# bartelvdh/Navtex

Hardware: AMD Instinct MI355X
Metric: IQ Msamples/s through FIR->FSK->bitsync (higher is better)
Workload: dtype f64

## Files before the change

navtex_amd/csrc/nvx_cascade.hip:

```cpp
#include <hip/hip_runtime.h>
#include <stdint.h>
#include <stdlib.h>
#include <mutex>

#include "nvx_cascade_wave.h"
#include "nvx_tune_table.h"

__device__ double2 nvx_tune_tab[NVX_TUNE_TAB_ENTRIES];

__device__ __forceinline__ int add_low_halves(unsigned a, unsigned b)
{
    int r;
    asm("v_add_u32_sdwa %0, sext(%1), sext(%2) dst_sel:DWORD dst_unused:UNUSED_PAD src0_sel:WORD_0 src1_sel:WORD_0"
        : "=v"(r) : "v"(a), "v"(b));
    return r;
}
__device__ __forceinline__ int add_high_halves(unsigned a, unsigned b)
{
    int r;
    asm("v_add_u32_sdwa %0, sext(%1), sext(%2) dst_sel:DWORD dst_unused:UNUSED_PAD src0_sel:WORD_1 src1_sel:WORD_1"
        : "=v"(r) : "v"(a), "v"(b));
    return r;
}
__device__ __forceinline__ double stage0_component(u32x4 v, bool odd)
{
    const int sI = add_low_halves(v.x, v.y) + add_low_halves(v.z, v.w);
    const int sQ = add_high_halves(v.x, v.y) + add_high_halves(v.z, v.w);
    int mine = (odd ? sQ : sI) + 4;
    const int other = odd ? sI : sQ;
    asm("" : "+v"(mine));
    const int tot = mine + dpp_swap_pairs(other);
    return (double)(tot >> 3);
}

struct Stage0Cic3 {
    unsigned sel_mine, sel_other;
    unsigned wa0, wa1, wb0, wb1, wc0, wc1;
    int c_prev, t_prev;
    bool last_pair;

    __device__ __forceinline__ void init(int lane)
    {
        const bool odd = lane & 1;
        sel_mine = odd ? 0x07060302u : 0x05040100u;
        sel_other = odd ? 0x05040100u : 0x07060302u;
        wa0 = odd ? (10u | 6u << 16) : (36u | 28u << 16);  wa1 = odd ? (3u | 1u << 16) : (21u | 15u << 16);
        wb0 = odd ? (48u | 48u << 16) : (28u | 36u << 16); wb1 = odd ? (46u | 42u << 16) : (42u | 46u << 16);
        wc0 = odd ? (6u | 10u << 16) : 0u;                 wc1 = odd ? (15u | 21u << 16) : (1u | 3u << 16);
        last_pair = lane >= 62;
        c_prev = 0; t_prev = 0;
    }
    __device__ __forceinline__ static int rot1(int v) { return __builtin_amdgcn_mov_dpp(v, 0x13C, 0xF, 0xF, false); }
    __device__ __forceinline__ static void dot2_first(nvx_short2 a, unsigned wb, unsigned wc, int &b, int &c)
    {
        asm("v_dot2_i32_i16 %0, %2, %3, 0\n\t"
            "v_dot2_i32_i16 %1, %2, %4, 0\n\t"
            "s_nop 2"
            : "=&v"(b), "=v"(c) : "v"(a), "v"(wb), "v"(wc));
    }
    __device__ __forceinline__ double step(u32x4 v)
    {
        const nvx_short2 m01 = as_short2(__builtin_amdgcn_perm(v.y, v.x, sel_mine)), m23 = as_short2(__builtin_amdgcn_perm(v.w, v.z, sel_mine));
        const nvx_short2 o01 = as_short2(__builtin_amdgcn_perm(v.y, v.x, sel_other)), o23 = as_short2(__builtin_amdgcn_perm(v.w, v.z, sel_other));
        int oa = __builtin_amdgcn_sdot2(o01, as_short2(wa0), 256, false); oa = __builtin_amdgcn_sdot2(o23, as_short2(wa1), oa, false);
        int ob, oc;
        dot2_first(o01, wb0, wc0, ob, oc);
        ob = __builtin_amdgcn_sdot2(o23, as_short2(wb1), ob, false); oc = __builtin_amdgcn_sdot2(o23, as_short2(wc1), oc, false);
        int A = dpp_swap_pairs(oa); A = __builtin_amdgcn_sdot2(m01, as_short2(wa0), A, false); A = __builtin_amdgcn_sdot2(m23, as_short2(wa1), A, false);
        int B = dpp_swap_pairs(ob); B = __builtin_amdgcn_sdot2(m01, as_short2(wb0), B, false); B = __builtin_amdgcn_sdot2(m23, as_short2(wb1), B, false);
        int C = dpp_swap_pairs(oc); C = __builtin_amdgcn_sdot2(m01, as_short2(wc0), C, false); C = __builtin_amdgcn_sdot2(m23, as_short2(wc1), C, false);
        const int t = B + rot1(rot1(last_pair ? c_prev : C));
        const int y = A + rot1(rot1(last_pair ? t_prev : t));
        c_prev = C; t_prev = t;
        return (double)(y >> 9);
    }
};

template <bool RAW>
__device__ __forceinline__ void load_pass(u32x4 (&pf)[RAW ? 8 : 1], const u32x4 *src)
{
    if (RAW) {
#pragma unroll
        for (int j = 0; j < 8; j++) pf[j] = __builtin_nontemporal_load(src + 64 * j);
    } else {
        pf[0] = __builtin_nontemporal_load(src);
    }
}

#define NVX_SPIN_LIMIT (1 << 22)

template <bool RAW, int NCH, int S0, typename ARGS, bool LIST = false>
__device__ __forceinline__ void cascade_wave_main(ARGS a)
{
    __shared__ CascadeLds<NCH> lds;
    const int lane = threadIdx.x;
    CascadeWave<NCH> cw;
    cw.init(&lds, lane);

    const size_t pass_words = RAW ? 2048 : 256;
    const size_t pass_stride = pass_words / 4;
    constexpr int NPF = RAW ? 8 : 1;
    const int half = lane >> 1, comp = lane & 1;
    const bool odd = lane & 1;
    double *xw = (double *)&lds.X[(half & 7) * XS + XH + (lane >> 4)] + comp;
    double2 *xw4 = &lds.X[(lane & 1) * 4 * XS + XH + half];
    static_assert(S0 == 1 || (S0 == 3 && RAW), "the third-order stage 0 belongs to the raw-rate kernels");
    Stage0Cic3 s0;
    if (S0 == 3) s0.init(lane);
    const int n_full = a.n_streams * a.split_from;
    const int n_units = n_full + 3 * a.n_streams * (a.n_frames - a.split_from);

    for (;;) {
        int u = 0;
        if (lane == 0) u = __hip_atomic_fetch_add(a.queue, 1, __ATOMIC_RELAXED, __HIP_MEMORY_SCOPE_AGENT);
        u = __builtin_amdgcn_readfirstlane(u);
        if (u >= n_units) break;
        int tpart, thirds, entry;
        if (u < n_full) { const int frame = u / a.n_streams; entry = u - frame * a.n_streams; tpart = 3 * frame; thirds = 3; }
        else { const int v = u - n_full, q = v / a.n_streams; entry = v - q * a.n_streams; tpart = 3 * a.split_from + q; thirds = 1; }
        const int part = tpart;
        int stream = entry;
        const uint8_t *state_rd = a.state[0];
        uint8_t *state_wr = a.state[1];
        unsigned third0 = a.third0;
        if (LIST) {
            const unsigned long long e = nvx_load_const_u64(a.part + entry);
            stream = (int)(unsigned)e;
            if (e >> 32) { state_rd = a.state[1]; state_wr = a.state[0]; }
            third0 = (unsigned)(nvx_load_const_u64(&a.part[entry].g0) / NVX_THIRD_Y3);
        }
        int *const done = a.done + entry;
        const unsigned mask = a.chain_masks[stream];

        bool preroll = a.independent && part > 0;
        bool late_publish = false;
        const u32x4 *unit0 = (const u32x4 *)(a.iq + ((size_t)stream * a.pitch + a.first_sample)) + (size_t)part * NVX_THIRD_PASSES * pass_stride + lane;
        u32x4 pfA[NPF];
        if (!preroll) load_pass<RAW>(pfA, unit0);

        if (part > 0 && !a.independent) {
            int spins = 0, ok = 0;
            do {
                int d = 0;
                if (lane == 0) d = __hip_atomic_load(done, __ATOMIC_RELAXED, __HIP_MEMORY_SCOPE_AGENT);
                d = __builtin_amdgcn_readfirstlane(d);
                ok = d >= part;
                if (!ok && a.dynamic_preroll) break;
                if (!ok) __builtin_amdgcn_s_sleep(32);
            } while (!ok && ++spins < NVX_SPIN_LIMIT);
            if (!ok && a.dynamic_preroll) {
                preroll = true; late_publish = true;
                if (lane == 0) __hip_atomic_fetch_add(a.status + 2, 1, __ATOMIC_RELAXED, __HIP_MEMORY_SCOPE_AGENT);
            } else {
                if (spins > 0 && lane == 0) {
                    __hip_atomic_fetch_add(a.status + 1, spins, __ATOMIC_RELAXED, __HIP_MEMORY_SCOPE_AGENT);
                    __hip_atomic_fetch_add(a.status + 2, 1, __ATOMIC_RELAXED, __HIP_MEMORY_SCOPE_AGENT);
                }
                if (!ok) {
                    if (lane == 0) __hip_atomic_store(a.status, NVX_STATUS_TIMEOUT, __ATOMIC_RELAXED, __HIP_MEMORY_SCOPE_AGENT);
                    break;
                }
                asm volatile("" ::: "memory");
            }
        }

        double2 *st = (double2 *)(state_wr + (size_t)stream * NVX_CASCADE_STATE_BYTES);
        const double2 *st_in = (part == 0) ? (const double2 *)(state_rd + (size_t)stream * NVX_CASCADE_STATE_BYTES) : st;
#ifdef NVX_INJECT_STALE
        if (part > 0 && !preroll && (u % NVX_INJECT_STALE) == 0) st_in = (const double2 *)(state_rd + (size_t)stream * NVX_CASCADE_STATE_BYTES);
#endif
        cw.set_mask(mask);
        unsigned long long ct = 0;
        if (!preroll) {
            NVX_WAVE_LDS_FENCE();
            const unsigned long long sealed = seal_load(st_in);
            unsigned long long fold = cw.state_in(st_in);
            if (S0 == 3 && s0.last_pair) {
                ct = __hip_atomic_load((const unsigned long long *)(st_in + NVX_STATE_CIC3) + (lane & 1), __ATOMIC_RELAXED, __HIP_MEMORY_SCOPE_AGENT);
                fold ^= seal_rotc<37>(ct);
            }
            const unsigned third_in = third0 + (unsigned)part;
            if (third_in != 0 && !seal_ok(sealed, wave_fold64(fold), stream, third_in)) {
                if (part == 0) {
                    if (lane == 0) __hip_atomic_store(a.status, NVX_STATUS_INTEGRITY, __ATOMIC_RELAXED, __HIP_MEMORY_SCOPE_AGENT);
                } else {
                    preroll = true; ct = 0;
                    if (lane == 0) __hip_atomic_fetch_add(a.status + 3, 1, __ATOMIC_RELAXED, __HIP_MEMORY_SCOPE_AGENT);
                }
            }
        }
        const int pre = preroll ? NVX_PREROLL_PASSES : 0;
        const int n_pass = pre + thirds * NVX_THIRD_PASSES;
        const u32x4 *src = unit0 - (size_t)pre * pass_stride;
        if (preroll) load_pass<RAW>(pfA, src);
        const u32x4 *nxt = src + pass_stride;
        cw.begin_unit(mask, a.y3, (size_t)(stream * 2) * a.y3_cap + a.y3_base + (size_t)part * NVX_THIRD_Y3, a.y3_cap,
                      ((part % 3) * (NVX_THIRD_PASSES * 64)) % NVX_MIX_N,
                      preroll ? NVX_PREROLL_U : 0, preroll ? NVX_PREROLL_Y2 : 0, !preroll);
        NVX_WAVE_LDS_FENCE();
        if (preroll) cw.state_zero();
        NVX_WAVE_LDS_FENCE();
        if (S0 == 3) { s0.c_prev = (int)(unsigned)ct; s0.t_prev = (int)(unsigned)(ct >> 32); }
        {
            const unsigned long long k01 = nvx_load_const_u64(a.tune_k + 2 * stream);
            int o_first = (part % 3) * (NVX_THIRD_PASSES * 64) - pre * 64;
            if (o_first < 0) o_first += NVX_PASSES_PER_FRAME * 64;
            cw.begin_table_mix((int)(unsigned)k01, (int)(unsigned)(k01 >> 32), o_first);
        }

        auto body = [&](u32x4 (&pf)[NPF], const int pass) {
            cw.tune_fetch(nvx_tune_tab);
            if (RAW) {
#pragma unroll
                for (int j = 0; j < 8; j++) xw[j * 8] = (S0 == 3) ? s0.step(pf[j]) : stage0_component(pf[j], odd);
            } else {
                const uint32_t w[4] = { pf[0].x, pf[0].y, pf[0].z, pf[0].w };
#pragma unroll
                for (int r = 0; r < 4; r++) {
                    double2 v;
                    v.x = (double)(int)(short)(w[r] & 0xffffu);
                    v.y = (double)((int)w[r] >> 16);
                    xw4[r * XS] = v;
                }
            }
            cw.tune_ready();
            if (pass + 1 < n_pass) load_pass<RAW>(pf, nxt);
            nxt += pass_stride;
            NVX_WAVE_LDS_FENCE();
            cw.compute_pass(true);
        };

        for (int pass = 0; pass < n_pass; pass++) {
            if (pass == pre) { cw.emit = true; cw.n3_done = 0; }
            body(pfA, pass);
        }

        NVX_WAVE_LDS_FENCE();
        if (late_publish) {
            int spins = 0, ok = 0;
            do {
                int d = 0;
                if (lane == 0) d = __hip_atomic_load(done, __ATOMIC_RELAXED, __HIP_MEMORY_SCOPE_AGENT);
                d = __builtin_amdgcn_readfirstlane(d);
                ok = d >= part;
                if (!ok) __builtin_amdgcn_s_sleep(32);
            } while (!ok && ++spins < NVX_SPIN_LIMIT);
            if (spins > 0 && lane == 0) __hip_atomic_fetch_add(a.status + 1, spins, __ATOMIC_RELAXED, __HIP_MEMORY_SCOPE_AGENT);
            if (!ok) {
                if (lane == 0) __hip_atomic_store(a.status, NVX_STATUS_TIMEOUT, __ATOMIC_RELAXED, __HIP_MEMORY_SCOPE_AGENT);
                break;
            }
            asm volatile("" ::: "memory");
        }
        if (!a.independent || part + thirds == 3 * a.n_frames) {
            unsigned long long fold = cw.state_out(st);
            if (S0 == 3 && s0.last_pair) {
                const unsigned long long ct_out = (unsigned long long)(unsigned)s0.c_prev | ((unsigned long long)(unsigned)s0.t_prev << 32);
                __hip_atomic_store((unsigned long long *)(st + NVX_STATE_CIC3) + (lane & 1), ct_out, __ATOMIC_RELAXED, __HIP_MEMORY_SCOPE_AGENT);
                fold ^= seal_rotc<37>(ct_out);
            }
            fold = wave_fold64(fold);
            if (lane == 0) seal_store(st, fold, stream, third0 + (unsigned)(part + thirds));
        }
        asm volatile("s_waitcnt vmcnt(0)" ::: "memory");
        if (lane == 0 && !a.independent) __hip_atomic_store(done, part + thirds, __ATOMIC_RELAXED, __HIP_MEMORY_SCOPE_AGENT);
    }
}

template <bool RAW, int NCH>
__global__ __launch_bounds__(64) void nvx_fir_cascade(nvx_cascade_args a)
{
    if (RAW) cascade_wave_main<RAW, NCH, 1, const nvx_cascade_args &>(a);
    else cascade_wave_main<RAW, NCH, 1, const nvx_cascade_args>(a);
}

__global__ __launch_bounds__(64) __attribute__((amdgpu_waves_per_eu(3, 3))) void nvx_fir_cascade_cic3_1(nvx_cascade_args a) { cascade_wave_main<true, 1, 3, const nvx_cascade_args &>(a); }
__global__ __launch_bounds__(64) void nvx_fir_cascade_cic3_2(nvx_cascade_args a) { cascade_wave_main<true, 2, 3, const nvx_cascade_args &>(a); }

template <bool RAW, int NCH, int S0>
__global__ __launch_bounds__(64) void nvx_fir_cascade_list(nvx_cascade_args a)
{
    if (RAW) cascade_wave_main<RAW, NCH, S0, const nvx_cascade_args &, true>(a);
    else cascade_wave_main<RAW, NCH, S0, const nvx_cascade_args, true>(a);
}

template <bool RAW, int NCH, int S0, bool LIST> struct CascadeKernel { static constexpr auto fn = nvx_fir_cascade_list<RAW, NCH, S0>; };
template <bool RAW, int NCH> struct CascadeKernel<RAW, NCH, 1, false> { static constexpr auto fn = nvx_fir_cascade<RAW, NCH>; };
template <> struct CascadeKernel<true, 1, 3, false> { static constexpr auto fn = nvx_fir_cascade_cic3_1; };
template <> struct CascadeKernel<true, 2, 3, false> { static constexpr auto fn = nvx_fir_cascade_cic3_2; };

#define NVX_MAX_DEVICES 64
static int env_int(const char *name, int dflt) { const char *e = getenv(name); return e ? atoi(e) : dflt; }

template <bool RAW, int NCH, int S0 = 1, bool LIST = false>
static hipError_t launch_cascade_as(const nvx_cascade_args *a, hipStream_t s)
{
    static std::mutex mu;
    static int cus_of[NVX_MAX_DEVICES], fit_of[NVX_MAX_DEVICES];
    int n_cus = 0, fit_per_cu = 0;
    {
        int dev = 0;
        hipError_t e = hipGetDevice(&dev);
        if (e != hipSuccess) return e;
        std::lock_guard<std::mutex> lk(mu);
        const bool cached = dev >= 0 && dev < NVX_MAX_DEVICES && cus_of[dev] > 0;
        if (!cached) {
            int cus = 0, per_cu = 0;
            e = hipDeviceGetAttribute(&cus, hipDeviceAttributeMultiprocessorCount, dev);
            if (e == hipSuccess) e = hipOccupancyMaxActiveBlocksPerMultiprocessor(&per_cu, CascadeKernel<RAW, NCH, S0, LIST>::fn, 64, 0);
            if (e != hipSuccess) return e;
            n_cus = cus; fit_per_cu = per_cu > 0 ? per_cu : 1;
            if (dev >= 0 && dev < NVX_MAX_DEVICES) { cus_of[dev] = n_cus; fit_of[dev] = fit_per_cu; }
        } else {
            n_cus = cus_of[dev]; fit_per_cu = fit_of[dev];
        }
    }
    int per_cu = fit_per_cu;
    if (a->max_waves_per_cu > 0 && a->max_waves_per_cu < per_cu) per_cu = a->max_waves_per_cu;
    if (a->max_waves_per_cu < 0 && per_cu + a->max_waves_per_cu >= 4) per_cu += a->max_waves_per_cu;
    const int resident = n_cus * per_cu;
    nvx_cascade_args args = *a;
    static const int force = env_int("NVX_INDEPENDENT", -1);
    args.independent = force >= 0 ? force : (a->n_streams < resident && a->n_frames > 1);
    const long long whole_units = (long long)a->n_streams * a->n_frames;
    const int split_frames = whole_units > resident ? 1 : ((args.independent && 3 * whole_units <= resident) ? a->n_frames : 0);
    args.split_from = a->n_frames - split_frames;
    const long long units = (long long)a->n_streams * (args.split_from + 3LL * split_frames);
    const unsigned grid = (unsigned)(units < resident ? units : resident);
    static const int dynamic = env_int("NVX_DYNAMIC_PREROLL", 1);
    args.dynamic_preroll = dynamic != 0;
    hipLaunchKernelGGL((CascadeKernel<RAW, NCH, S0, LIST>::fn), dim3(grid), dim3(64), 0, s, args);
    return hipGetLastError();
}

static hipError_t tune_table_ready()
{
    static std::mutex mu;
    static bool done[NVX_MAX_DEVICES];
    int dev = 0;
    hipError_t e = hipGetDevice(&dev);
    if (e != hipSuccess) return e;
    if (dev < 0 || dev >= NVX_MAX_DEVICES) return hipErrorInvalidDevice;
    std::lock_guard<std::mutex> lk(mu);
    if (done[dev]) return hipSuccess;
    double2 *tab = (double2 *)calloc(NVX_TUNE_TAB_ENTRIES, sizeof(double2));
    if (!tab) return hipErrorOutOfMemory;
    for (int j = 0; j < NVX_TUNE_TAB_N; j++) nvx_tune_entry(j, &tab[j].x, &tab[j].y);
    for (int o = 0; o < NVX_MIX_N; o++) {
        const int j = (NVX_TUNE_NOMINAL_K * o) % NVX_TUNE_TAB_N;
        tab[NVX_TUNE_TAB_N + j] = double2{ NVX_MIX_CR[o], NVX_MIX_CI[o] };
        tab[2 * NVX_TUNE_TAB_N + (NVX_TUNE_TAB_N - j) % NVX_TUNE_TAB_N] = double2{ NVX_MIX_CR[o], -NVX_MIX_CI[o] };
    }
    e = hipMemcpyToSymbol(HIP_SYMBOL(nvx_tune_tab), tab, NVX_TUNE_TAB_ENTRIES * sizeof(double2), 0, hipMemcpyHostToDevice);
    free(tab);
    if (e == hipSuccess) done[dev] = true;
    return e;
}

extern "C" hipError_t nvx_launch_cascade(const nvx_cascade_args *a, int raw, int nch, hipStream_t s)
{
    { hipError_t e = tune_table_ready(); if (e != hipSuccess) return e; }
    hipError_t e = hipMemsetAsync(a->queue, 0, (size_t)(NVX_CASCADE_CTRL_INTS + a->n_streams) * sizeof(int), s);
    if (e != hipSuccess) return e;
    const bool cic3 = raw && a->stage0_order == 3;
    if (a->part) {
        if (cic3) return nch == 1 ? launch_cascade_as<true, 1, 3, true>(a, s) : launch_cascade_as<true, 2, 3, true>(a, s);
        if (raw) return nch == 1 ? launch_cascade_as<true, 1, 1, true>(a, s) : launch_cascade_as<true, 2, 1, true>(a, s);
        return nch == 1 ? launch_cascade_as<false, 1, 1, true>(a, s) : launch_cascade_as<false, 2, 1, true>(a, s);
    }
    if (cic3) return nch == 1 ? launch_cascade_as<true, 1, 3>(a, s) : launch_cascade_as<true, 2, 3>(a, s);
    if (raw) return nch == 1 ? launch_cascade_as<true, 1>(a, s) : launch_cascade_as<true, 2>(a, s);
    return nch == 1 ? launch_cascade_as<false, 1>(a, s) : launch_cascade_as<false, 2>(a, s);
}
```

navtex_amd/csrc/nvx_cascade_wave.h:

```cpp
#ifndef NVX_CASCADE_WAVE_H
#define NVX_CASCADE_WAVE_H

#include <hip/hip_runtime.h>
#include <stdint.h>

#include "nvx_tables.h"
#include "nvx_kernels.h"
#include "nvx_device.h"

#define XPH 8
#define XH 5
#define XS 37
#define X_ENTRIES (XPH * XS)
#define NVX_Y2_RUN 160

template <int NCH> struct Geo;
template <> struct Geo<1> { static constexpr int U_RUN = 224, Y2_PER_RUN = 32, Y2_RUN = NVX_Y2_RUN, Y3_PER_RUN = NVX_Y2_RUN / 10, U_PEND_MAX = 256, U_LEFT_MAX = 32; };
template <> struct Geo<2> { static constexpr int U_RUN = 112, Y2_PER_RUN = 16, Y2_RUN = 80, Y3_PER_RUN = 8, U_PEND_MAX = 160, U_LEFT_MAX = 48; };
template <int NCH> struct GeoSizes {
    static constexpr int U_ENTRIES = ((46 + Geo<NCH>::U_PEND_MAX) + 7) / 8 * 8;
    static constexpr int Y2_ENTRIES = ((70 + Geo<NCH>::Y2_RUN) + 7) / 8 * 8;
};
static_assert(Geo<1>::Y2_RUN % Geo<1>::Y2_PER_RUN == 0 && Geo<2>::Y2_RUN % Geo<2>::Y2_PER_RUN == 0, "NVX_Y2_RUN: a whole number of FIR2 runs (160)");
static_assert(Geo<1>::U_RUN % 32 == 0 && Geo<2>::U_RUN % 16 == 0 && 46 + Geo<1>::U_LEFT_MAX <= 128 && 46 + Geo<2>::U_LEFT_MAX <= 128, "slide covers two rows of 64");

template <int NCH, bool F3IN> struct CascadeLdsY2 { double2 Y2[NCH][GeoSizes<NCH>::Y2_ENTRIES]; };
template <int NCH> struct CascadeLdsY2<NCH, false> {};
template <int NCH, bool F3IN = true>
struct CascadeLds : CascadeLdsY2<NCH, F3IN> {
    double2 X[X_ENTRIES];
    double2 U[NCH][GeoSizes<NCH>::U_ENTRIES];
    double2 mix[2][2 * NVX_MIX_N];
};

__device__ __forceinline__ int dpp_swap_pairs(int v)
{
    return __builtin_amdgcn_mov_dpp(v, 0xB1, 0xF, 0xF, true);
}
__device__ __forceinline__ double dpp_swap_pairs_f64(double v)
{
    return __hiloint2double(dpp_swap_pairs(__double2hiint(v)), dpp_swap_pairs(__double2loint(v)));
}

#define NVX_F1_GROUP 4
#define NVX_F1_AHEAD 3
#define NVX_F23_AHEAD 12
__device__ __forceinline__ constexpr int f1_offset(int j)
{
    const int t = 7 - j, r = t & 7, fl = (t - r) / 8;
    return 2 * (r * XS + fl);
}

template <int N> struct TapIndex {
    int first[N];
    constexpr TapIndex(const double (&h)[N]) : first{}
    {
        for (int i = 0; i < N; i++) {
            int f = i;
            for (int k = 0; k < i; k++) if (h[k] == h[i]) { f = k; break; }
            first[i] = f;
        }
    }
};
static constexpr TapIndex<NVX_T1> NVX_H1_FIRST(NVX_H1);

__device__ __forceinline__ double2 state_load(const double2 *p)
{
    double2 r;
    r.x = __hip_atomic_load(&p->x, __ATOMIC_RELAXED, __HIP_MEMORY_SCOPE_AGENT);
    r.y = __hip_atomic_load(&p->y, __ATOMIC_RELAXED, __HIP_MEMORY_SCOPE_AGENT);
    return r;
}
__device__ __forceinline__ void state_store(double2 *p, double2 v)
{
    __hip_atomic_store(&p->x, v.x, __ATOMIC_RELAXED, __HIP_MEMORY_SCOPE_AGENT);
    __hip_atomic_store(&p->y, v.y, __ATOMIC_RELAXED, __HIP_MEMORY_SCOPE_AGENT);
}

template <int R> __device__ __forceinline__ unsigned long long seal_rotc(unsigned long long v)
{
    constexpr int r = R & 63;
    if constexpr (r == 0) return v;
    else return (v << r) | (v >> (64 - r));
}
template <int SLOT> __device__ __forceinline__ unsigned long long seal_pair(double2 v)
{
    return seal_rotc<14 * SLOT + 3>((unsigned long long)__double_as_longlong(v.x)) ^ seal_rotc<14 * SLOT + 10>((unsigned long long)__double_as_longlong(v.y));
}
__device__ __forceinline__ unsigned long long seal_tag(int stream, unsigned third)
{
    unsigned long long t = ((unsigned long long)(unsigned)stream << 32) | third;
    t *= 0x9E3779B97F4A7C15ull; t ^= t >> 29; t *= 0xBF58476D1CE4E5B9ull; t ^= t >> 32;
    return t;
}
template <int CTRL, int R> __device__ __forceinline__ unsigned long long seal_step(unsigned long long v)
{
    const unsigned lo = (unsigned)__builtin_amdgcn_mov_dpp((int)(unsigned)v, CTRL, 0xF, 0xF, true);
    const unsigned hi = (unsigned)__builtin_amdgcn_mov_dpp((int)(unsigned)(v >> 32), CTRL, 0xF, 0xF, true);
    return v ^ seal_rotc<R>(((unsigned long long)hi << 32) | lo);
}
__device__ __forceinline__ unsigned long long seal_row(unsigned lo, unsigned hi, int lane0)
{
    return ((unsigned long long)(unsigned)__builtin_amdgcn_readlane((int)hi, lane0) << 32) | (unsigned)__builtin_amdgcn_readlane((int)lo, lane0);
}
__device__ __forceinline__ unsigned long long wave_fold64(unsigned long long v)
{
    v = seal_step<0xB1, 1>(v);
    v = seal_step<0x4E, 2>(v);
    v = seal_step<0x141, 4>(v);
    v = seal_step<0x140, 8>(v);
    const unsigned lo = (unsigned)v, hi = (unsigned)(v >> 32);
    return seal_row(lo, hi, 0) ^ seal_rotc<16>(seal_row(lo, hi, 16)) ^ seal_rotc<32>(seal_row(lo, hi, 32)) ^ seal_rotc<48>(seal_row(lo, hi, 48));
}
__device__ __forceinline__ void seal_store(double2 *st, unsigned long long fold, int stream, unsigned third)
{
    unsigned long long *p = (unsigned long long *)(st + NVX_STATE_SEAL);
    __hip_atomic_store(p, fold ^ seal_tag(stream, third), __ATOMIC_RELAXED, __HIP_MEMORY_SCOPE_AGENT);
    __hip_atomic_store(p + 1, ((unsigned long long)(unsigned)stream << 32) | third, __ATOMIC_RELAXED, __HIP_MEMORY_SCOPE_AGENT);
}
__device__ __forceinline__ unsigned long long seal_load(const double2 *st_in)
{
    return __hip_atomic_load((const unsigned long long *)(st_in + NVX_STATE_SEAL), __ATOMIC_RELAXED, __HIP_MEMORY_SCOPE_AGENT);
}
__device__ __forceinline__ bool seal_ok(unsigned long long got, unsigned long long fold, int stream, unsigned third)
{
    const unsigned long long d = got ^ fold ^ seal_tag(stream, third);
    return __builtin_amdgcn_readfirstlane((int)((unsigned)d | (unsigned)(d >> 32))) == 0;
}

template <int NCH, bool F3IN = true>
struct CascadeWave {
    CascadeLds<NCH, F3IN> *lds;
    int lane, half, comp;
    const lds_vdouble *xrv;
    const lds_vd2 *mixrow;
    int lane_mod9;
    double h1v[NVX_T1];
    unsigned mask;
    int chain_of_slot0;
    int n_u, n_y2, n3_done, mixbase;
    nvx_d2 mix_next;
    bool emit;
    double2 *y3; size_t y3_row0, y3_cap;
    double2 *y2_lane; int n2_done;
    int toff[NCH], tk[NCH], tidx[NCH];
    nvx_d2 tc[NCH];

    __device__ __forceinline__ void init(CascadeLds<NCH, F3IN> *l, int lane_)
    {
        lds = l; lane = lane_; half = lane >> 1; comp = lane & 1;
        xrv = (const lds_vdouble *)((const double *)&lds->X[XH + half] + comp);
        lane_mod9 = (2 * half) % 9;
        if (!F3IN && lane < 4 * NVX_MIX_N) {
            const int j9 = lane % NVX_MIX_N;
            double cr = 0.0, ci = 0.0;
#pragma unroll
            for (int j = 0; j < NVX_MIX_N; j++) if (j9 == j) { cr = NVX_MIX_CR[j]; ci = NVX_MIX_CI[j]; }
            lds->mix[0][lane % (2 * NVX_MIX_N)] = double2{ cr, ci };
            lds->mix[1][lane % (2 * NVX_MIX_N)] = double2{ cr, -ci };
        }
#pragma unroll
        for (int i = 0; i < NVX_T1; i++)
            if (NVX_H1_FIRST.first[i] == i) { h1v[i] = NVX_H1[i]; asm volatile("" : "+v"(h1v[i])); }
    }

    __device__ __forceinline__ void set_mask(unsigned chain_mask)
    {
        mask = chain_mask;
        chain_of_slot0 = (NCH == 1) ? ((mask & 1u) ? 0 : 1) : 0;
    }
    __device__ __forceinline__ void begin_unit(unsigned chain_mask, double2 *y3_, size_t row0, size_t cap, int mixbase0, int n_u0, int n_y20, bool emit0)
    {
        set_mask(chain_mask);
        mixrow = (const lds_vd2 *)&lds->mix[(comp ^ (NCH == 1 ? chain_of_slot0 : 0)) ? 0 : 1][lane_mod9];
        y3 = y3_; y3_row0 = row0; y3_cap = cap;
        mixbase = mixbase0; n_u = n_u0; n_y2 = n_y20; n3_done = 0; n2_done = 0; emit = emit0;
        if (!F3IN) mix_next = mixrow[mixbase];
    }

    __device__ __forceinline__ void begin_table_mix(int k0, int k1, int o_first)
    {
        int o = o_first + lane;
        if (o >= NVX_TUNE_TAB_N) o -= NVX_TUNE_TAB_N;
#pragma unroll
        for (int c = 0; c < NCH; c++) {
            const int ch = __builtin_amdgcn_readfirstlane((NCH == 1) ? chain_of_slot0 : c);
            const int k = ch ? k1 : k0;
            const bool nominal = k == (ch ? -NVX_TUNE_NOMINAL_K : NVX_TUNE_NOMINAL_K);
            tk[c] = ((k % NVX_TUNE_TAB_N) + NVX_TUNE_TAB_N) % NVX_TUNE_TAB_N;
            toff[c] = nominal ? NVX_TUNE_TAB_N * (1 + ch) : 0;
            tidx[c] = (tk[c] * o) % NVX_TUNE_TAB_N;
        }
    }
    __device__ __forceinline__ void tune_fetch(const double2 *tab)
    {
#pragma unroll
        for (int c = 0; c < NCH; c++) {
            tc[c] = *(const nvx_d2 *)(tab + toff[c] + tidx[c]);
            tidx[c] += (64 * tk[c]) % NVX_TUNE_TAB_N;
            if (tidx[c] >= NVX_TUNE_TAB_N) tidx[c] -= NVX_TUNE_TAB_N;
        }
    }

    __device__ __forceinline__ void tune_ready()
    {
#pragma unroll
        for (int c = 0; c < NCH; c++) asm volatile("" :: "v"(tc[c].x), "v"(tc[c].y));
    }

    __device__ __forceinline__ void begin_unit_y2(double2 *y2buf, size_t pitch, int row0, int row1, size_t first)
    {
        const int ch = (NCH == 1) ? chain_of_slot0 : (lane >> 5);
        const int row = ch ? row1 : row0;
        y2_lane = row < 0 ? nullptr : y2buf + ((size_t)row * pitch + NVX_Y2_PREFIX + first);
    }

    __device__ __forceinline__ unsigned long long state_in(const double2 *st_in)
    {
        unsigned long long f = 0;
        if (lane < 36) {
            const int v = lane + 4;
            const double2 x = state_load(st_in + lane);
            f ^= seal_pair<0>(x);
            lds->X[(v & 7) * XS + (v >> 3)] = x;
        }
#pragma unroll
        for (int c = 0; c < NCH; c++) {
            const int ch = (NCH == 1) ? chain_of_slot0 : c;
            const double2 *su = st_in + 36 + ch * (46 + 70);
            if (lane < 46) { const double2 u = state_load(su + lane); f ^= (c ? seal_pair<4>(u) : seal_pair<1>(u)); lds->U[c][lane] = u; }
            if constexpr (F3IN) {
                const double2 y = state_load(su + 46 + lane);
                f ^= (c ? seal_pair<5>(y) : seal_pair<2>(y));
                lds->Y2[c][lane] = y;
                if (lane < 6) { const double2 t = state_load(su + 46 + 64 + lane); f ^= (c ? seal_pair<6>(t) : seal_pair<3>(t)); lds->Y2[c][64 + lane] = t; }
            }
        }
        return f;
    }
    __device__ __forceinline__ void state_zero()
    {
        const double2 zero = { 0.0, 0.0 };
        if (lane < XPH * XH) lds->X[(lane & 7) * XS + (lane >> 3)] = zero;
#pragma unroll
        for (int c = 0; c < NCH; c++) {
            for (int i = lane; i < 46 + NVX_PREROLL_U; i += 64) lds->U[c][i] = zero;
            if constexpr (F3IN) for (int i = lane; i < 70 + NVX_PREROLL_Y2; i += 64) lds->Y2[c][i] = zero;
        }
    }
    __device__ __forceinline__ unsigned long long state_out(double2 *st)
    {
        unsigned long long f = 0;
        if (lane < 36) {
            const int v = lane + 4;
            const double2 x = lds->X[(v & 7) * XS + (v >> 3)];
            f ^= seal_pair<0>(x);
            state_store(st + lane, x);
        }
#pragma unroll
        for (int c = 0; c < NCH; c++) {
            const int ch = (NCH == 1) ? chain_of_slot0 : c;
            double2 *su = st + 36 + ch * (46 + 70);
            if (lane < 46) { const double2 u = lds->U[c][lane]; f ^= (c ? seal_pair<4>(u) : seal_pair<1>(u)); state_store(su + lane, u); }
            if constexpr (F3IN) {
                const double2 y = lds->Y2[c][lane];
                f ^= (c ? seal_pair<5>(y) : seal_pair<2>(y));
                state_store(su + 46 + lane, y);
                if (lane < 6) { const double2 t = lds->Y2[c][64 + lane]; f ^= (c ? seal_pair<6>(t) : seal_pair<3>(t)); state_store(su + 46 + 64 + lane, t); }
            }
        }
        return f;
    }

    __device__ __forceinline__ void compute_pass(const bool table_mix = false)
    {
        nvx_d2 c0 = { 0.0, 0.0 }, c1 = { 0.0, 0.0 };
        if (!table_mix) { c0 = mix_next; c1 = mixrow[mixbase + 1]; mix_next = c1; }
        nvx_d2 tail = { 0.0, 0.0 };
        if (lane < XPH * XH) tail = *(const lds_vd2 *)&lds->X[(lane & 7) * XS + 32 + (lane >> 3)];
        double xs[NVX_T1 + 4];
        constexpr int F1N = NVX_T1 + 4, F1NG = (F1N + NVX_F1_GROUP - 1) / NVX_F1_GROUP;
#pragma unroll
        for (int j = 0; j < NVX_F1_AHEAD * NVX_F1_GROUP; j++) xs[j] = xrv[f1_offset(j)];
        double a0 = 0.0, a1 = 0.0;
#pragma unroll
        for (int g = 0; g < F1NG; g++) {
            if (g + NVX_F1_AHEAD < F1NG) {
                NVX_PIN_AFTER(a1);
#pragma unroll
                for (int j = (g + NVX_F1_AHEAD) * NVX_F1_GROUP; j < (g + NVX_F1_AHEAD + 1) * NVX_F1_GROUP && j < F1N; j++) xs[j] = xrv[f1_offset(j)];
            }
            const int lo = g * NVX_F1_GROUP, hi = (lo + NVX_F1_GROUP < F1N ? lo + NVX_F1_GROUP : F1N) - 1;
            if (hi > lo) asm volatile("" : "+v"(xs[lo]) : "v"(xs[hi]));
#pragma unroll
            for (int j = lo; j <= hi; j++) {
                if (j < NVX_T1) a1 += h1v[NVX_H1_FIRST.first[j]] * xs[j];
                if (j >= 4) a0 += h1v[NVX_H1_FIRST.first[j - 4]] * xs[j];
            }
        }
        if (table_mix) {
            const double o0 = dpp_swap_pairs_f64(a0), o1 = dpp_swap_pairs_f64(a1);
#pragma unroll
            for (int c = 0; c < NCH; c++) {
                const nvx_d2 tp = { dpp_swap_pairs_f64(tc[c].x), dpp_swap_pairs_f64(tc[c].y) };
                const nvx_d2 c0t = comp ? tp : tc[c], c1t = comp ? tc[c] : tp;
                const double A0 = a0 * c0t.x, A1 = a1 * c1t.x;
                const double B0 = o0 * c0t.y, B1 = o1 * c1t.y;
                double *uw = (double *)&lds->U[c][46 + n_u + 2 * half] + comp;
                uw[0] = comp ? A0 + B0 : A0 - B0;
                uw[2] = comp ? A1 + B1 : A1 - B1;
            }
        } else {
            const double o0 = dpp_swap_pairs_f64(a0), o1 = dpp_swap_pairs_f64(a1);
            const double A0 = a0 * c0.x, A1 = a1 * c1.x;
            const double B0 = o0 * c0.y, B1 = o1 * c1.y;
#pragma unroll
            for (int c = 0; c < NCH; c++) {
                const int ch = (NCH == 1) ? chain_of_slot0 : c;
                double *uw = (double *)&lds->U[c][46 + n_u + 2 * half] + comp;
                uw[0] = (NCH == 1 || ch == 0) ? A0 + B0 : A0 - B0;
                uw[2] = (NCH == 1 || ch == 0) ? A1 + B1 : A1 - B1;
            }
        }
        n_u += 64;
        if (!table_mix) { mixbase += 1; if (mixbase == NVX_MIX_N) mixbase = 0; }
        NVX_WAVE_LDS_FENCE();
        if (lane < XPH * XH) *(lds_vd2 *)&lds->X[(lane & 7) * XS + (lane >> 3)] = tail;
        NVX_WAVE_LDS_FENCE();

        constexpr int U_RUN = Geo<NCH>::U_RUN, Y2_PER_RUN = Geo<NCH>::Y2_PER_RUN;
        constexpr int Y2_RUN = Geo<NCH>::Y2_RUN, Y3_PER_RUN = Geo<NCH>::Y3_PER_RUN;
        const int f2c = (NCH == 2) ? (lane >> 5) : 0;
        const int f2o = (NCH == 2) ? ((lane >> 1) & 15) : half;
        constexpr int UT1 = 46 + Geo<NCH>::U_LEFT_MAX - 64;
        while (n_u >= U_RUN) {
            nvx_d2 ut0[NCH], ut1[NCH];
#pragma unroll
            for (int c = 0; c < NCH; c++) {
                ut0[c] = *(const lds_vd2 *)&lds->U[c][U_RUN + lane];
                ut1[c] = *(const lds_vd2 *)&lds->U[c][U_RUN + 64 + (lane < UT1 ? lane : UT1 - 1)];
            }
            {
                const lds_vdouble *ub = (const lds_vdouble *)((const double *)&lds->U[f2c][7 * f2o] + comp);
                double xs2[NVX_T2], acc = 0.0;
#pragma unroll
                for (int i = 0; i < NVX_F23_AHEAD; i++) xs2[i] = ub[2 * (52 - i)];
                nvx_static_for<0, NVX_T2>([&](auto ic) {
                    constexpr int i = decltype(ic)::value;
                    if constexpr (i + NVX_F23_AHEAD < NVX_T2) { NVX_PIN_AFTER(acc); xs2[i + NVX_F23_AHEAD] = ub[2 * (52 - (i + NVX_F23_AHEAD))]; }
                    acc += NVX_H2[i] * xs2[i];
                });
                if constexpr (F3IN) {
                    if (NCH == 1 || ((mask >> f2c) & 1u)) ((double *)&lds->Y2[f2c][70 + n_y2 + f2o])[comp] = acc;
                } else {
                    if (emit && y2_lane) ((double *)(y2_lane + n2_done + f2o))[comp] = acc;
                }
            }
            NVX_WAVE_LDS_FENCE();
            const int keep = 46 + n_u - U_RUN;
#pragma unroll
            for (int c = 0; c < NCH; c++) {
                if (lane < keep) *(lds_vd2 *)&lds->U[c][lane] = ut0[c];
                if (lane + 64 < keep) *(lds_vd2 *)&lds->U[c][64 + lane] = ut1[c];
            }
            NVX_WAVE_LDS_FENCE();
            n_u -= U_RUN;
            if constexpr (!F3IN) { if (emit) n2_done += Y2_PER_RUN; continue; }
            n_y2 += Y2_PER_RUN;

            if constexpr (F3IN) if (n_y2 >= Y2_RUN) {
                const int f3c = (NCH == 2) ? ((lane >> 4) & 1) : 0;
                const int f3o = half & (Y3_PER_RUN - 1);
                const bool f3live = lane < 2 * Y3_PER_RUN * NCH;
                nvx_d2 yt0[NCH], yt1[NCH];
#pragma unroll
                for (int c = 0; c < NCH; c++) {
                    yt0[c] = *(const lds_vd2 *)&lds->Y2[c][Y2_RUN + lane];
                    yt1[c] = *(const lds_vd2 *)&lds->Y2[c][Y2_RUN + 64 + (lane < 6 ? lane : 5)];
                }
                {
                    const int ch = (NCH == 1) ? chain_of_slot0 : f3c;
                    const lds_vdouble *yb = (const lds_vdouble *)((const double *)&lds->Y2[f3c][10 * f3o] + comp);
                    double xs3[NVX_T3], acc = 0.0;
#pragma unroll
                    for (int i = 0; i < NVX_F23_AHEAD; i++) xs3[i] = yb[2 * (79 - i)];
                    nvx_static_for<0, NVX_T3>([&](auto ic) {
                        constexpr int i = decltype(ic)::value;
                        if constexpr (i + NVX_F23_AHEAD < NVX_T3) { NVX_PIN_AFTER(acc); xs3[i + NVX_F23_AHEAD] = yb[2 * (79 - (i + NVX_F23_AHEAD))]; }
                        acc += NVX_H3[i] * xs3[i];
                    });
                    if (emit && f3live && (NCH == 1 || ((mask >> f3c) & 1u))) {
                        double *out = (double *)(y3 + (y3_row0 + (size_t)ch * y3_cap + n3_done + f3o));
                        out[comp] = acc;
                    }
                }
                NVX_WAVE_LDS_FENCE();
                const int keep3 = 70 + n_y2 - Y2_RUN;
#pragma unroll
                for (int c = 0; c < NCH; c++) {
                    if (lane < keep3) *(lds_vd2 *)&lds->Y2[c][lane] = yt0[c];
                    if (lane + 64 < keep3) *(lds_vd2 *)&lds->Y2[c][64 + lane] = yt1[c];
                }
                NVX_WAVE_LDS_FENCE();
                n_y2 -= Y2_RUN;
                n3_done += Y3_PER_RUN;
            }
        }
    }
};

#endif
```

Before: 1.526 million.

## Stage nominal-tune mixer coefficients in LDS and skip per-pass table fetches

When both chains use the nominal tuning constant, the mixer coefficients are periodic with NVX_MIX_N. They are now preloaded once into a per-channel LDS row, and the per-pass global table fetch is skipped. In the non-nominal case the fetched coefficients go through LDS instead of DPP swaps, and the sign selection becomes a precomputed sign-bit XOR, which removes the per-channel DPP shuffles and selects. In exchange there are extra LDS traffic and fences, and the LDS mix array is resized per kernel variant under a static residency check.

After: 1.506 million. -1.3%, worse.

```diff
diff --git a/navtex_amd/csrc/nvx_cascade.hip b/navtex_amd/csrc/nvx_cascade.hip
--- a/navtex_amd/csrc/nvx_cascade.hip
+++ b/navtex_amd/csrc/nvx_cascade.hip
@@ -88,6 +88,12 @@
 }
 
 #define NVX_SPIN_LIMIT (1 << 22)
+
+__device__ __forceinline__ void status_raise(int *status, int code)
+{
+    asm volatile("" : "+v"(code));
+    __hip_atomic_store(status, code, __ATOMIC_RELAXED, __HIP_MEMORY_SCOPE_AGENT);
+}
 
 template <bool RAW, int NCH, int S0, typename ARGS, bool LIST = false>
 __device__ __forceinline__ void cascade_wave_main(ARGS a)
@@ -157,7 +163,7 @@
                     __hip_atomic_fetch_add(a.status + 2, 1, __ATOMIC_RELAXED, __HIP_MEMORY_SCOPE_AGENT);
                 }
                 if (!ok) {
-                    if (lane == 0) __hip_atomic_store(a.status, NVX_STATUS_TIMEOUT, __ATOMIC_RELAXED, __HIP_MEMORY_SCOPE_AGENT);
+                    if (lane == 0) status_raise(a.status, NVX_STATUS_TIMEOUT);
                     break;
                 }
                 asm volatile("" ::: "memory");
@@ -182,7 +188,7 @@
             const unsigned third_in = third0 + (unsigned)part;
             if (third_in != 0 && !seal_ok(sealed, wave_fold64(fold), stream, third_in)) {
                 if (part == 0) {
-                    if (lane == 0) __hip_atomic_store(a.status, NVX_STATUS_INTEGRITY, __ATOMIC_RELAXED, __HIP_MEMORY_SCOPE_AGENT);
+                    if (lane == 0) status_raise(a.status, NVX_STATUS_INTEGRITY);
                 } else {
                     preroll = true; ct = 0;
                     if (lane == 0) __hip_atomic_fetch_add(a.status + 3, 1, __ATOMIC_RELAXED, __HIP_MEMORY_SCOPE_AGENT);
@@ -205,7 +211,7 @@
             const unsigned long long k01 = nvx_load_const_u64(a.tune_k + 2 * stream);
             int o_first = (part % 3) * (NVX_THIRD_PASSES * 64) - pre * 64;
             if (o_first < 0) o_first += NVX_PASSES_PER_FRAME * 64;
-            cw.begin_table_mix((int)(unsigned)k01, (int)(unsigned)(k01 >> 32), o_first);
+            cw.begin_table_mix(nvx_tune_tab, (int)(unsigned)k01, (int)(unsigned)(k01 >> 32), o_first);
         }
 
         auto body = [&](u32x4 (&pf)[NPF], const int pass) {
@@ -247,7 +253,7 @@
             } while (!ok && ++spins < NVX_SPIN_LIMIT);
             if (spins > 0 && lane == 0) __hip_atomic_fetch_add(a.status + 1, spins, __ATOMIC_RELAXED, __HIP_MEMORY_SCOPE_AGENT);
             if (!ok) {
-                if (lane == 0) __hip_atomic_store(a.status, NVX_STATUS_TIMEOUT, __ATOMIC_RELAXED, __HIP_MEMORY_SCOPE_AGENT);
+                if (lane == 0) status_raise(a.status, NVX_STATUS_TIMEOUT);
                 break;
             }
             asm volatile("" ::: "memory");
diff --git a/navtex_amd/csrc/nvx_cascade_wave.h b/navtex_amd/csrc/nvx_cascade_wave.h
--- a/navtex_amd/csrc/nvx_cascade_wave.h
+++ b/navtex_amd/csrc/nvx_cascade_wave.h
@@ -12,6 +12,7 @@
 #define XH 5
 #define XS 37
 #define X_ENTRIES (XPH * XS)
+#define NVX_MIX_ROWS 64
 #define NVX_Y2_RUN 160
 
 template <int NCH> struct Geo;
@@ -26,12 +27,15 @@
 
 template <int NCH, bool F3IN> struct CascadeLdsY2 { double2 Y2[NCH][GeoSizes<NCH>::Y2_ENTRIES]; };
 template <int NCH> struct CascadeLdsY2<NCH, false> {};
+template <int NCH, bool F3IN> struct CascadeLdsMix { typedef double2 type[NCH][NVX_MIX_ROWS]; };
+template <int NCH> struct CascadeLdsMix<NCH, false> { typedef double2 type[2][2 * NVX_MIX_N]; };
 template <int NCH, bool F3IN = true>
 struct CascadeLds : CascadeLdsY2<NCH, F3IN> {
     double2 X[X_ENTRIES];
     double2 U[NCH][GeoSizes<NCH>::U_ENTRIES];
-    double2 mix[2][2 * NVX_MIX_N];
+    typename CascadeLdsMix<NCH, F3IN>::type mix;
 };
+static_assert(11 * sizeof(CascadeLds<1>) <= 160 * 1024 && 8 * sizeof(CascadeLds<2>) <= 160 * 1024, "LDS residency of the single-wave cascade kernels");
 
 __device__ __forceinline__ int dpp_swap_pairs(int v)
 {
@@ -134,6 +138,7 @@
     int lane, half, comp;
     const lds_vdouble *xrv;
     const lds_vd2 *mixrow;
+    int mixoff;
     int lane_mod9;
     double h1v[NVX_T1];
     unsigned mask;
@@ -143,15 +148,17 @@
     bool emit;
     double2 *y3; size_t y3_row0, y3_cap;
     double2 *y2_lane; int n2_done;
+    int mixstep;
     int toff[NCH], tk[NCH], tidx[NCH];
     nvx_d2 tc[NCH];
+    unsigned bsign[NCH];
 
     __device__ __forceinline__ void init(CascadeLds<NCH, F3IN> *l, int lane_)
     {
         lds = l; lane = lane_; half = lane >> 1; comp = lane & 1;
         xrv = (const lds_vdouble *)((const double *)&lds->X[XH + half] + comp);
         lane_mod9 = (2 * half) % 9;
-        if (!F3IN && lane < 4 * NVX_MIX_N) {
+        if constexpr (!F3IN) if (lane < 4 * NVX_MIX_N) {
             const int j9 = lane % NVX_MIX_N;
             double cr = 0.0, ci = 0.0;
 #pragma unroll
@@ -172,28 +179,54 @@
     __device__ __forceinline__ void begin_unit(unsigned chain_mask, double2 *y3_, size_t row0, size_t cap, int mixbase0, int n_u0, int n_y20, bool emit0)
     {
         set_mask(chain_mask);
-        mixrow = (const lds_vd2 *)&lds->mix[(comp ^ (NCH == 1 ? chain_of_slot0 : 0)) ? 0 : 1][lane_mod9];
+        if constexpr (!F3IN) mixrow = (const lds_vd2 *)&lds->mix[(comp ^ (NCH == 1 ? chain_of_slot0 : 0)) ? 0 : 1][lane_mod9];
         y3 = y3_; y3_row0 = row0; y3_cap = cap;
         mixbase = mixbase0; n_u = n_u0; n_y2 = n_y20; n3_done = 0; n2_done = 0; emit = emit0;
-        if (!F3IN) mix_next = mixrow[mixbase];
-    }
-
-    __device__ __forceinline__ void begin_table_mix(int k0, int k1, int o_first)
-    {
-        int o = o_first + lane;
+        if constexpr (!F3IN) mix_next = mixrow[mixbase];
+    }
+
+    __device__ __forceinline__ void begin_table_mix(const double2 *tab, int k0, int k1, int o_first)
+    {
+        int ln = lane;
+        asm volatile("" : "+v"(ln));
+        int o = o_first + ln;
         if (o >= NVX_TUNE_TAB_N) o -= NVX_TUNE_TAB_N;
+        bool all_nominal = true;
+        int chs[NCH];
 #pragma unroll
         for (int c = 0; c < NCH; c++) {
             const int ch = __builtin_amdgcn_readfirstlane((NCH == 1) ? chain_of_slot0 : c);
             const int k = ch ? k1 : k0;
             const bool nominal = k == (ch ? -NVX_TUNE_NOMINAL_K : NVX_TUNE_NOMINAL_K);
+            all_nominal = all_nominal && nominal;
+            chs[c] = ch;
             tk[c] = ((k % NVX_TUNE_TAB_N) + NVX_TUNE_TAB_N) % NVX_TUNE_TAB_N;
             toff[c] = nominal ? NVX_TUNE_TAB_N * (1 + ch) : 0;
-            tidx[c] = (tk[c] * o) % NVX_TUNE_TAB_N;
-        }
+        }
+        mixstep = __builtin_amdgcn_readfirstlane(all_nominal ? 1 : 0);
+        if (mixstep == 0) {
+            mixoff = (ln & ~1) * (int)sizeof(double2);
+            mixbase = 0;
+#pragma unroll
+            for (int c = 0; c < NCH; c++) {
+                tidx[c] = (tk[c] * o) % NVX_TUNE_TAB_N;
+                bsign[c] = (unsigned)((ln & 1) ^ 1) << 31;
+            }
+        } else {
+            mixoff = ((ln & ~1) % NVX_MIX_N) * (int)sizeof(double2);
+#pragma unroll
+            for (int c = 0; c < NCH; c++) bsign[c] = (unsigned)((ln & 1) ^ chs[c] ^ 1) << 31;
+            if (ln < 2 * NVX_MIX_N) {
+                const nvx_d2 e = *(const nvx_d2 *)(tab + NVX_TUNE_TAB_N + (NVX_TUNE_NOMINAL_K * (ln % NVX_MIX_N)) % NVX_TUNE_TAB_N);
+#pragma unroll
+                for (int c = 0; c < NCH; c++) *(lds_vd2 *)&lds->mix[c][ln] = e;
+            }
+        }
+        NVX_WAVE_LDS_FENCE();
     }
     __device__ __forceinline__ void tune_fetch(const double2 *tab)
     {
+        if (mixstep != 0) return;
 #pragma unroll
         for (int c = 0; c < NCH; c++) {
             tc[c] = *(const nvx_d2 *)(tab + toff[c] + tidx[c]);
@@ -204,6 +237,7 @@
 
     __device__ __forceinline__ void tune_ready()
     {
+        if (mixstep != 0) return;
 #pragma unroll
         for (int c = 0; c < NCH; c++) asm volatile("" :: "v"(tc[c].x), "v"(tc[c].y));
     }
@@ -240,7 +274,9 @@
     }
     __device__ __forceinline__ void state_zero()
     {
-        const double2 zero = { 0.0, 0.0 };
+        double z0 = 0.0;
+        if constexpr (F3IN) asm volatile("" : "+v"(z0));
+        const double2 zero = { z0, z0 };
         if (lane < XPH * XH) lds->X[(lane & 7) * XS + (lane >> 3)] = zero;
 #pragma unroll
         for (int c = 0; c < NCH; c++) {
@@ -276,6 +312,13 @@
     {
         nvx_d2 c0 = { 0.0, 0.0 }, c1 = { 0.0, 0.0 };
         if (!table_mix) { c0 = mix_next; c1 = mixrow[mixbase + 1]; mix_next = c1; }
+        nvx_d2 r0[NCH], r1[NCH];
+        if (table_mix && mixstep == 0) {
+            int ln = lane;
+            asm volatile("" : "+v"(ln));
+#pragma unroll
+            for (int c = 0; c < NCH; c++) *(lds_vd2 *)&lds->mix[c][ln] = tc[c];
+        }
         nvx_d2 tail = { 0.0, 0.0 };
         if (lane < XPH * XH) tail = *(const lds_vd2 *)&lds->X[(lane & 7) * XS + 32 + (lane >> 3)];
         double xs[NVX_T1 + 4];
@@ -290,6 +333,14 @@
 #pragma unroll
                 for (int j = (g + NVX_F1_AHEAD) * NVX_F1_GROUP; j < (g + NVX_F1_AHEAD + 1) * NVX_F1_GROUP && j < F1N; j++) xs[j] = xrv[f1_offset(j)];
             }
+            if (table_mix && g + NVX_F1_AHEAD == F1NG) {
+                NVX_PIN_AFTER(a1);
+#pragma unroll
+                for (int c = 0; c < NCH; c++) {
+                    const lds_vd2 *row = (const lds_vd2 *)((const char *)&lds->mix[c][0] + (mixoff + mixbase * (int)sizeof(double2)));
+                    r0[c] = row[0]; r1[c] = row[1];
+                }
+            }
             const int lo = g * NVX_F1_GROUP, hi = (lo + NVX_F1_GROUP < F1N ? lo + NVX_F1_GROUP : F1N) - 1;
             if (hi > lo) asm volatile("" : "+v"(xs[lo]) : "v"(xs[hi]));
 #pragma unroll
@@ -302,13 +353,11 @@
             const double o0 = dpp_swap_pairs_f64(a0), o1 = dpp_swap_pairs_f64(a1);
 #pragma unroll
             for (int c = 0; c < NCH; c++) {
-                const nvx_d2 tp = { dpp_swap_pairs_f64(tc[c].x), dpp_swap_pairs_f64(tc[c].y) };
-                const nvx_d2 c0t = comp ? tp : tc[c], c1t = comp ? tc[c] : tp;
-                const double A0 = a0 * c0t.x, A1 = a1 * c1t.x;
-                const double B0 = o0 * c0t.y, B1 = o1 * c1t.y;
+                const double A0 = a0 * r0[c].x, A1 = a1 * r1[c].x;
+                const double B0 = o0 * r0[c].y, B1 = o1 * r1[c].y;
                 double *uw = (double *)&lds->U[c][46 + n_u + 2 * half] + comp;
-                uw[0] = comp ? A0 + B0 : A0 - B0;
-                uw[2] = comp ? A1 + B1 : A1 - B1;
+                uw[0] = A0 + __hiloint2double(__double2hiint(B0) ^ (int)bsign[c], __double2loint(B0));
+                uw[2] = A1 + __hiloint2double(__double2hiint(B1) ^ (int)bsign[c], __double2loint(B1));
             }
         } else {
             const double o0 = dpp_swap_pairs_f64(a0), o1 = dpp_swap_pairs_f64(a1);
@@ -324,6 +373,7 @@
         }
         n_u += 64;
         if (!table_mix) { mixbase += 1; if (mixbase == NVX_MIX_N) mixbase = 0; }
+        else { mixbase += mixstep; if (mixbase == NVX_MIX_N) mixbase = 0; }
         NVX_WAVE_LDS_FENCE();
         if (lane < XPH * XH) *(lds_vd2 *)&lds->X[(lane & 7) * XS + (lane >> 3)] = tail;
         NVX_WAVE_LDS_FENCE();
```
